# gmum/3d-point-clouds-autocomplete

Hardware: AMD Instinct MI355X
Metric: train-step point-clouds/sec at B=64, N=2048 (Chamfer+EMD) (higher is better)
Workload: dtype f32 storage / accumulation / results; matrix products formed from f16 x2 (bf16 x3) pieces of the fp32 operands — NOT IEEE-fp32 products: the all-fp32-kernel step is `value_strict_fp32`

## Files before the change

3d-point-clouds-autocomplete_amd/csrc/conv_pp.hip:

```cpp
#include "hp_common.h"
#include "hp_conv_split.h"
#include <algorithm>
#include <cstdlib>
#include <type_traits>

namespace {

typedef _Float16 f16x8 __attribute__((ext_vector_type(8)));
typedef _Float16 f16x4 __attribute__((ext_vector_type(4)));
typedef _Float16 f16x2 __attribute__((ext_vector_type(2)));
typedef float f32x16 __attribute__((ext_vector_type(16)));
typedef float f32x4 __attribute__((ext_vector_type(4)));
typedef unsigned int u32x4 __attribute__((ext_vector_type(4)));
typedef unsigned int u32x2 __attribute__((ext_vector_type(2)));

constexpr int kTarget = 14;
constexpr int kExpMax = HP_PP_EXP_MAX;

__device__ __forceinline__ int frexp_exp(unsigned bits) {
    const int E = (int)((bits >> 23) & 0xff);
    return E ? E - 126 : 0;
}
__device__ __forceinline__ float pow2f(int e) {
    e = max(-126, min(127, e));
// ... 356 lines not shown
                        L[q + 1][pr] = s2[1];
                    }
                    if (row < M) {
                        *reinterpret_cast<u32x4*>(line + q * 16) = u32x4{H[q][0], H[q][1], H[q + 1][0], H[q + 1][1]};
                        *reinterpret_cast<u32x4*>(line + 64 + q * 16) = u32x4{L[q][0], L[q][1], L[q + 1][0], L[q + 1][1]};
                    }
                }
            }
        }
        __syncthreads();
    }
}

__global__ __launch_bounds__(256) void conv1_pp_kernel(const float* __restrict__ x, long sXz, const float* __restrict__ W, long sWz,
                                                       const float* __restrict__ b, long sBz, _Float16* __restrict__ h, int* __restrict__ hexp,
                                                       long sWs, long R) {
    __shared__ float smax[4];
    const int z = blockIdx.y;
    x += z * sXz; W += z * sWz; b += z * sBz;
    unsigned char* hb = reinterpret_cast<unsigned char*>(h) + z * sWs * 4;
    hexp += z * sWs;
    const int c4 = (threadIdx.x & 15) * 4;
    float w0[4], w1[4], w2[4], bb[4];
#pragma unroll
    for (int u = 0; u < 4; ++u) {
        w0[u] = W[(c4 + u) * 3];
        w1[u] = W[(c4 + u) * 3 + 1];
        w2[u] = W[(c4 + u) * 3 + 2];
        bb[u] = b[c4 + u];
    }
    for (long tile = blockIdx.x; tile * 128 < R; tile += gridDim.x) {
        const long base = tile * 128 + (threadIdx.x >> 4);
        float xv[8][3];
#pragma unroll
        for (int q = 0; q < 8; ++q) {
            const long row = min(base + 16 * q, R - 1);
            xv[q][0] = x[row * 3];
            xv[q][1] = x[row * 3 + 1];
            xv[q][2] = x[row * 3 + 2];
        }
        float o[8][4];
        float m = 0.f;
#pragma unroll
        for (int q = 0; q < 8; ++q)
#pragma unroll
            for (int u = 0; u < 4; ++u) {
// ... 138 lines not shown

}

bool hp_conv_presplit_enabled() { return g_presplit.get() != 0; }
int hp_conv_pp_ncb(int l) {
    static const int kC[5] = {0, 64, 128, 256, 512};
    return l <= 1 ? 1 : kC[l] / pp_bn(kC[l]);
}
HP_API int hp_conv_presplit_set(int on) { return g_presplit.set(on); }

static inline long pexp_off(int l, long tp) { return hp_conv_pp_exp_offset(l, tp); }

long hp_conv_pp_fmt_offset(long R) { return hp_conv_pp_exp_offset(5, hp_conv_split_tiles_pad(R)); }

int hp_conv_pp_layer1(int n, const float* x, long sXz, const float* W, long sWz, const float* b, long sBz, float* h1, float* area0,
                      long sWs, long R, hipStream_t stream) {
    const long tp = hp_conv_split_tiles_pad(R), blocks = (R + 127) / 128;
    hipLaunchKernelGGL(conv1_pp_kernel, dim3((unsigned)(blocks < 2048 ? blocks : 2048), n), dim3(256), 0, stream, x, sXz, W, sWz, b, sBz,
                       reinterpret_cast<_Float16*>(h1), reinterpret_cast<int*>(area0 + pexp_off(1, tp)), sWs, R);
    HP_RETURN_LAST_ERROR();
}

int hp_conv_pp_layer(int l, int n, const float* X, const float* bias, long sBiasz, float* C, float* area0, long sWs, long M,
                     float* cmax, int* cidx, int group_rows, hipStream_t stream) {
    static const int kRowsL[5] = {0, 128, 384, 896, 1408};
    static const long kWOffL[4] = {0, 8192, 40960, 172032};
    static const int kKL[4] = {64, 128, 256, 512};
    if (l < 2 || l > 5 || M <= 0) return -1;
    const long tp = hp_conv_split_tiles_pad(M);
    PpParams p{};
    p.A = reinterpret_cast<const _Float16*>(X);
    p.aexp = reinterpret_cast<const int*>(area0 + pexp_off(l - 1, tp));
    p.K = kKL[l - 2];
    p.a_ncb = hp_conv_pp_ncb(l - 1);
// ... 117 lines not shown
```

3d-point-clouds-autocomplete_amd/csrc/conv_split.hip:

```cpp
#include "hp_common.h"
#include "hp_conv_split.h"

namespace {

typedef _Float16 f16x8 __attribute__((ext_vector_type(8)));
typedef _Float16 f16x4 __attribute__((ext_vector_type(4)));
typedef float f32x16 __attribute__((ext_vector_type(16)));
typedef float f32x4 __attribute__((ext_vector_type(4)));
typedef unsigned int u32x4 __attribute__((ext_vector_type(4)));

constexpr int BM = 128, BN = 128, BK = 32, ROW = BK;
constexpr int kTarget = 14;

__device__ __forceinline__ int frexp_exp(unsigned bits) {
    const int E = (int)((bits >> 23) & 0xff);
    return E ? E - 126 : 0;
}
__device__ __forceinline__ float pow2f(int e) {
    e = max(-126, min(127, e));
    return __uint_as_float((unsigned)(e + 127) << 23);
}

struct PrepParams {
    const float* W[4];
    long sWz[4];
    _Float16* hl;
    int* wexp;
    unsigned* amax;
    long n_amax;
    long sArea;
    int* fmt;
    int fmt_value;
};
constexpr int kRows[5] = {0, 128, 384, 896, 1408};
constexpr long kWOff[4] = {0, 8192, 40960, 172032};
constexpr int kK[4] = {64, 128, 256, 512};

__global__ __launch_bounds__(256) void conv_split_prep_kernel(const PrepParams p) {
    const int z = blockIdx.y, lane = threadIdx.x & 63;
    const int row = blockIdx.x * 4 + (threadIdx.x >> 6);
    for (long i = (long)blockIdx.x * 256 + threadIdx.x; i < p.n_amax; i += (long)gridDim.x * 256) p.amax[z * p.sArea + i] = 0u;
    if (blockIdx.x == 0 && threadIdx.x == 0) p.fmt[z * p.sArea] = p.fmt_value;
    int l = 0;
    while (l < 3 && row >= kRows[l + 1]) ++l;
    const int n = row - kRows[l], K = kK[l];
    const float* w = p.W[l] + z * p.sWz[l] + (long)n * K;
    float v[8];
    float m = 0.f;
#pragma unroll
    for (int u = 0; u < 8; ++u) {
        const int k = lane + 64 * u;
        v[u] = k < K ? w[k] : 0.f;
        m = fmaxf(m, fabsf(v[u]));
    }
#pragma unroll
    for (int o = 32; o > 0; o >>= 1) m = fmaxf(m, __shfl_xor(m, o, 64));
    const int e = kTarget - frexp_exp(__float_as_uint(m));
    const float s = pow2f(e);
    _Float16* hl = p.hl + 2 * z * p.sArea + 2 * kWOff[l] + (long)n * 2 * K;
#pragma unroll
    for (int u = 0; u < 8; ++u) {
        const int k = lane + 64 * u;
        if (k < K) {
            const float xs = v[u] * s;
            const _Float16 hh = (_Float16)xs;
            hl[(k >> 5) * 64 + (k & 31)] = hh;
            hl[(k >> 5) * 64 + 32 + (k & 31)] = (_Float16)(xs - (float)hh);
        }
    }
    if (lane == 0) p.wexp[z * p.sArea + row] = e;
}

__global__ __launch_bounds__(256) void conv1_kernel(const float* __restrict__ x, long sXz, const float* __restrict__ W, long sWz,
                                                    const float* __restrict__ b, long sBz, float* __restrict__ h, long sHz,
                                                    unsigned* __restrict__ amax, long sAz, long R) {
    __shared__ float smax[4];
    const int z = blockIdx.y;
    x += z * sXz; W += z * sWz; b += z * sBz; h += z * sHz;
    const int c4 = (threadIdx.x & 15) * 4;
    float w0[4], w1[4], w2[4], bb[4];
#pragma unroll
    for (int u = 0; u < 4; ++u) {
        w0[u] = W[(c4 + u) * 3];
        w1[u] = W[(c4 + u) * 3 + 1];
        w2[u] = W[(c4 + u) * 3 + 2];
// ... 278 lines not shown
            out[(k >> 5) * 64 + (k & 31)] = hh;
            out[(k >> 5) * 64 + 32 + (k & 31)] = (_Float16)(xs - (float)hh);
        }
    }
    if (lane == 0) wexp[row] = e;
}

hp::Switch g_split("HP_CONV_SPLIT", 1);

}

long hp_conv_split_area_floats(long R) { return HP_CS_AMAX_OFF + 20 * hp_conv_split_tiles_pad(R) + 4; }
bool hp_conv_split_enabled() { return g_split.get() != 0; }
HP_API int hp_conv_split_set(int on) { return g_split.set(on); }

int hp_conv_split_prep(int n, const float* const* W0, const float* const* W1, float* area0, long sArea, long R, int fmt, hipStream_t stream) {
    PrepParams p{};
    for (int l = 0; l < 4; ++l) {
        p.W[l] = W0[l];
        p.sWz[l] = n > 1 ? (long)(W1[l] - W0[l]) : 0;
    }
    p.amax = reinterpret_cast<unsigned*>(area0 + HP_CS_AMAX_OFF);
    p.n_amax = 4 * hp_conv_split_tiles_pad(R);
    p.wexp = reinterpret_cast<int*>(area0 + HP_CS_WEXP_OFF);
    p.hl = reinterpret_cast<_Float16*>(area0 + HP_CS_HI_OFF);
    p.sArea = sArea;
    p.fmt = reinterpret_cast<int*>(area0 + hp_conv_pp_fmt_offset(R));
    p.fmt_value = fmt;
    hipLaunchKernelGGL(conv_split_prep_kernel, dim3(kRows[4] / 4, n), dim3(256), 0, stream, p);
    HP_RETURN_LAST_ERROR();
}

int hp_conv_split_layer1(int n, const float* x, long sXz, const float* W, long sWz, const float* b, long sBz, float* h1, long sHz,
                         float* area0, long sArea, long R, hipStream_t stream) {
    const long blocks = (R + 127) / 128;
    hipLaunchKernelGGL(conv1_kernel, dim3((unsigned)(blocks < 2048 ? blocks : 2048), n), dim3(256), 0, stream, x, sXz, W, sWz, b,
                       sBz, h1, sHz, reinterpret_cast<unsigned*>(area0 + HP_CS_AMAX_OFF), sArea, R);
    HP_RETURN_LAST_ERROR();
}

int hp_conv_split_layer(int l, int n, const float* X, long sXz, const float* bias, long sBiasz, float* C, long sCz, float* area0,
                        long sArea, long M, int relu, int colmax, float* cmax, int* cidx, int group_rows, hipStream_t stream) {
    if (l < 2 || l > 5 || M <= 0) return -1;
    CsParams p{};
// ... 55 lines not shown
```

3d-point-clouds-autocomplete_amd/csrc/heads_fwd.hip:

```cpp
#include "hp_common.h"
#include <algorithm>
#include <cstdlib>
#include <type_traits>

namespace {

typedef __bf16 bf16x8 __attribute__((ext_vector_type(8)));
typedef float f32x4 __attribute__((ext_vector_type(4)));
typedef unsigned int u32x4 __attribute__((ext_vector_type(4)));

constexpr int kK = 2048, kSteps = kK / 32;
constexpr int kWaves = 5, kThreads = kWaves * 64;
constexpr int kT5Step = 12 * 1024;
constexpr int kG = 2, kStages = kSteps / kG;
constexpr int kT5Ring = 3, kWRing = 4;
constexpr int kT5Stage = kG * kT5Step;
constexpr int kWStage = kWaves * kG * 2048;
constexpr int kLds = kT5Ring * kT5Stage + kWRing * kWStage;
constexpr long kT5Bytes = (long)kSteps * kT5Step;

__device__ __forceinline__ void split3(const float (&x)[8], bf16x8& p1, bf16x8& p2, bf16x8& p3) {
    u32x4 a, b, c;
#pragma unroll
    for (int i = 0; i < 4; ++i) {
        const float x0 = x[2 * i], x1 = x[2 * i + 1];
        const float h0 = __uint_as_float(__float_as_uint(x0) & 0xffff0000u), h1 = __uint_as_float(__float_as_uint(x1) & 0xffff0000u);
        const float r0 = x0 - h0, r1 = x1 - h1;
        const float m0 = __uint_as_float(__float_as_uint(r0) & 0xffff0000u), m1 = __uint_as_float(__float_as_uint(r1) & 0xffff0000u);
        const float s0 = r0 - m0, s1 = r1 - m1;
        a[i] = __builtin_amdgcn_perm(__float_as_uint(x1), __float_as_uint(x0), 0x07060302u);
        b[i] = __builtin_amdgcn_perm(__float_as_uint(r1), __float_as_uint(r0), 0x07060302u);
        c[i] = __builtin_amdgcn_perm(__float_as_uint(s1), __float_as_uint(s0), 0x07060302u);
    }
    p1 = __builtin_bit_cast(bf16x8, a);
    p2 = __builtin_bit_cast(bf16x8, b);
    p3 = __builtin_bit_cast(bf16x8, c);
}

__global__ __launch_bounds__(64) void heads_t5_split_kernel(int B, const float* __restrict__ t5, unsigned char* __restrict__ out) {
    const int s = blockIdx.x >> 2, ct = blockIdx.x & 3, lane = threadIdx.x, c = 16 * ct + (lane & 15), kg = lane >> 4;
    float x[8];
#pragma unroll
    for (int j = 0; j < 8; ++j) x[j] = 0.f;
    if (c < B) {
        const f32x4 v0 = *reinterpret_cast<const f32x4*>(t5 + (long)c * kK + 32 * s + 8 * kg);
        const f32x4 v1 = *reinterpret_cast<const f32x4*>(t5 + (long)c * kK + 32 * s + 8 * kg + 4);
#pragma unroll
        for (int j = 0; j < 4; ++j) {
            x[j] = v0[j];
            x[4 + j] = v1[j];
        }
    }
    bf16x8 p[3];
    split3(x, p[0], p[1], p[2]);
    unsigned char* dst = out + (long)s * kT5Step + (ct * 3) * 1024 + lane * 16;
#pragma unroll
    for (int q = 0; q < 3; ++q) *reinterpret_cast<bf16x8*>(dst + q * 1024) = p[q];
}

__device__ __forceinline__ void glds16(const void* sbase, unsigned voff, unsigned lds_dst) {
    unsigned keep;
// ... 98 lines not shown
    }
    asm volatile("s_waitcnt vmcnt(0)" ::: "memory");
}

hp::Switch g_heads_fwd("HP_HEADS_FWD", 1);

}

bool hp_heads_fwd_enabled() { return g_heads_fwd.get() != 0; }
int hp_heads_fwd_set(int on) { return g_heads_fwd.set(on); }
long hp_heads_fwd_ws_floats() { return kT5Bytes / 4; }
bool hp_heads_fwd_ok(int B, int N, int K, const float* t5, const float* W, const float* ws) {
    auto a16 = [](const void* p) { return (reinterpret_cast<uintptr_t>(p) & 15) == 0; };
    return B >= 1 && B <= 64 && K == kK && N >= 16 && (long)N * K * 4 < (1L << 32) && a16(t5) && a16(W) && a16(ws);
}
int hp_heads_fwd(int B, int N, const float* t5, const float* W, const float* bias, float* theta, int theta_ld, float* ws,
                 hipStream_t stream) {
    unsigned char* t5p = reinterpret_cast<unsigned char*>(ws);
    hipLaunchKernelGGL(heads_t5_split_kernel, dim3(kSteps * 4), dim3(64), 0, stream, B, t5, t5p);
    const int ntiles = (N + 15) / 16;
    const int grid = (ntiles + kWaves - 1) / kWaves;
    hipLaunchKernelGGL(heads_fwd_kernel, dim3(grid), dim3(kThreads), 0, stream, B, N, W, bias, t5p, theta, theta_ld);
    HP_RETURN_LAST_ERROR();
}
```

3d-point-clouds-autocomplete_amd/csrc/hp_conv_split.h:

```cpp
#pragma once
#include <hip/hip_runtime.h>

#define HP_CS_WEXP_OFF 0L
#define HP_CS_HI_OFF 1408L
#define HP_CS_LO_OFF (HP_CS_HI_OFF + 434176L / 2)
#define HP_CS_AMAX_OFF (HP_CS_LO_OFF + 434176L / 2)

#define HP_PP_EXP_MAX 54
#define HP_PP_FMT_F32 0
#define HP_PP_FMT_P 0x50464d54

inline long hp_conv_split_tiles_pad(long R) { return ((R + 127) / 128 + 3) / 4 * 4; }
long hp_conv_split_area_floats(long R);
bool hp_conv_split_enabled();
int hp_conv_split_prep(int n, const float* const* W0, const float* const* W1, float* area0, long sArea, long R, int fmt, hipStream_t stream);
int hp_conv_split_layer1(int n, const float* x, long sXz, const float* W, long sWz, const float* b, long sBz, float* h1, long sHz,
                         float* area0, long sArea, long R, hipStream_t stream);
int hp_conv_split_layer(int l, int n, const float* X, long sXz, const float* bias, long sBiasz, float* C, long sCz, float* area0,
                        long sArea, long M, int relu, int colmax, float* cmax, int* cidx, int group_rows, hipStream_t stream);

bool hp_conv_presplit_enabled();
long hp_conv_pp_fmt_offset(long R);
int hp_conv_pp_layer1(int n, const float* x, long sXz, const float* W, long sWz, const float* b, long sBz, float* h1, float* area0,
                      long sWs, long R, hipStream_t stream);
int hp_conv_pp_layer(int l, int n, const float* X, const float* bias, long sBiasz, float* C, float* area0, long sWs, long M,
                     float* cmax, int* cidx, int group_rows, hipStream_t stream);
int hp_conv_pp_mark(int n, float* area0, long sWs, long R, int fmt, hipStream_t stream);
int hp_conv_pp_unpack_ws(float* ws, long R, hipStream_t stream);
inline long hp_conv_pp_exp_offset(int l, long tp) { return HP_CS_AMAX_OFF + 4 * tp + (long)(l - 1) * 4 * tp; }
int hp_conv_pp_ncb(int l);
```

3d-point-clouds-autocomplete_amd/csrc/hp_model.h:

```cpp
#pragma once

#define HP_MAX_HEADS 8
#define HP_MAX_TN_LAYERS 8

typedef struct HpEncoderWeights {
    const float* conv_w[5];
    const float* conv_b[5];
    const float* fc_w;
    const float* fc_b;
    const float* mu_w;
    const float* mu_b;
    const float* std_w;
    const float* std_b;
} HpEncoderWeights;

typedef struct HpEncoderGrads {
    float* conv_w[5];
    float* conv_b[5];
    float* fc_w;
    float* fc_b;
    float* mu_w;
    float* mu_b;
    float* std_w;
    float* std_b;
// ... 52 lines not shown

enum { HP_HEADS_FWD_STREAM = 0, HP_HEADS_FWD_GEMM = 1, HP_HEADS_FWD_PER_HEAD = 2 };
enum { HP_HEADS_DW_DIRECT = 0, HP_HEADS_DW_GEMM = 1, HP_HEADS_DW_PER_HEAD = 2, HP_HEADS_DW_SKIPPED = 3 };
typedef struct HpHeadsPlan {
    int fwd_route;
    int dw_route;
    int dw_rows_route;
} HpHeadsPlan;

#ifdef __cplusplus
bool hp_heads_dw_fast_ok(int cols, const float* t5, const float* out);
bool hp_heads_fwd_enabled();
int hp_heads_fwd_set(int on);
long hp_heads_fwd_ws_floats();
bool hp_heads_fwd_ok(int B, int N, int K, const float* t5, const float* W, const float* ws);
int hp_heads_fwd(int B, int N, const float* t5, const float* W, const float* bias, float* theta, int theta_ld, float* ws,
                 hipStream_t stream);
int hp_heads_dw_launch(int Kc, int rows, int r0, const float* dtheta, int theta_ld, const float* t5, int cols, float* dW,
                       float* db, hipStream_t stream);
#endif
```

3d-point-clouds-autocomplete_amd/csrc/model.hip:

```cpp
#include "hp_common.h"
#include "hp_gemm.h"
#include "hp_conv_split.h"
#include "hp_model.h"
#include "hp_skinny.h"
#include "hp_enc_bwd.h"
#include <algorithm>
#include <cstdlib>

extern "C" int hp_gemm_f32(const HpGemmDesc* d, hipStream_t stream);
extern "C" int hp_gemm_tile_rows(const HpGemmDesc* d);
extern "C" int hp_colsum_f32(int batch, int M, int N, const float* X, long sXz, int ldx, const float* mask, long sMaskz,
                             int ldmask, float* out, long sOz, float* ws, hipStream_t stream);

namespace {

constexpr int kEnc[6] = {3, 64, 128, 256, 512, 512};
constexpr int kTrunk[5] = {64, 128, 512, 1024, 2048};
constexpr long kSplitWs = 4L << 20;

#define TRY(x)            \
    do {                  \
        int _rc = (x);    \
        if (_rc) return _rc; \
    } while (0)

inline long cdiv(long a, long b) { return (a + b - 1) / b; }

int pick_ksplit(int outM, int outN, int kc, int batch) {
    const long tiles = cdiv(outM, 64) * cdiv(outN, 64) * batch;
    if (tiles >= 512 || kc < 256) return 1;
    long ks = tiles >= 256 ? std::min<long>(cdiv(768, tiles), kc / 512)
                           : std::min<long>(cdiv(512, tiles), kc / 128);
    ks = std::max<long>(1, std::min<long>(ks, (long)outM * outN * batch <= 8192 ? 128 : 64));
    while (ks > 1 && (long)outM * outN * batch * ks > kSplitWs) --ks;
    return (int)ks;
}

struct Op {
    hipStream_t s;
    float* splitws;
    const int* dyn = nullptr;
// ... 300 lines not shown
        }
        __syncthreads();
    }
}

__global__ __launch_bounds__(256) void vae_head_fwd_kernel(long n, const float* __restrict__ eps, const float* __restrict__ mu,
                                                           const float* __restrict__ lv, float* __restrict__ z, int out, int z_ld,
                                                           float* __restrict__ explv) {
    const long t = (long)blockIdx.x * 256 + threadIdx.x;
    if (t >= n) return;
    const float e = expf(lv[t]);
    explv[t] = e;
    z[(t / out) * z_ld + t % out] = __builtin_fmaf(eps[t], e, mu[t]);
}

__global__ __launch_bounds__(256) void vae_head_bwd_kernel(long n, const float* __restrict__ eps, const float* __restrict__ lv,
                                                           const float* __restrict__ gz, int out, int gz_ld,
                                                           const float* __restrict__ gmu, const float* __restrict__ gexplv,
                                                           float* __restrict__ dmu, float* __restrict__ dlv) {
    const long t = (long)blockIdx.x * 256 + threadIdx.x;
    if (t >= n) return;
    const float a = gz ? gz[(t / out) * gz_ld + t % out] : 0.f;
    dmu[t] = a + (gmu ? gmu[t] : 0.f);
    dlv[t] = (a * eps[t] + (gexplv ? gexplv[t] : 0.f)) * expf(lv[t]);
}

long enc_fwd_ws(long B, long Np) { return B * Np * (64 + 128 + 256 + 512 + 512) + hp_conv_split_area_floats(B * Np); }
long enc_bwd_ws(long B, long out) {
    const long Rc = B * 512;
    return Rc * 4 + Rc * (64 + 128 + 256 + 512) * 2 + B * (2 * out + 4 * 512) + kSplitWs + 64 + (B * (5 * 512 + 4) + 16) +
// ... 54 lines not shown
    }
    for (int e = 0; e < n && Sh > 1; ++e) {
        const HpEncoderWeights* w = t[e].w;
        float* hs = t[e].slabs + (long)S * 64 * 512;
        for (int hd = 0; hd < (t[e].is_vae ? 2 : 1); ++hd) {
            HpSkOp& op = pr.op[pr.nops++];
            op.type = HP_SK_FIN; op.phase = 2;
            op.a.p = hs + (long)hd * Sh * 64 * out_size; op.a.slab = 64L * out_size; op.a.S = Sh; op.a.ld = out_size;
            op.a.bias = hd ? w->std_b : w->mu_b;
            op.out = hd ? t[e].lv : t[e].mu; op.out_ld = hd ? out_size : t[e].mu_ld;
            op.M = B; op.N = out_size; op.K = 1;
        }
    }
    return 0;
}
int enc_tail_forward_skinny(int B, int out_size, int n, const EncTail* t, hipStream_t stream) {
    HpSkProgram pr;
    if (enc_tail_forward_program(B, out_size, n, t, pr)) return -2;
    return hp_skinny_run(&pr, stream);
}

struct EncTailBwd {
    const float *g, *f;
    const HpEncoderWeights* w;
    const float* dmu;
    int dmu_ld;
    const float* dlv;
    const HpEncoderGrads* gr;
    float *dfc, *dg, *slabs;
};
int enc_tail_backward_program(int B, int out_size, int n, const EncTailBwd* t, HpSkProgram& pr) {
    if (B > 64 || out_size % 32) return -2;
    pr = HpSkProgram{};
// ... 76 lines not shown
    d5.group_rows = Np;
    r.tr = r.split ? 128 : hp_gemm_tile_rows(&d5);
    r.tail_off = -1;
    r.fused = r.tr > 0 && Np % r.tr == 0;
    if (r.fused) {
        r.tiles = R / r.tr;
        if (R * 512 - up4(2 * r.tiles * 512) >= 4L * 64 * 512 + 8L * 64 * out_size) r.tail_off = up4(2 * r.tiles * 512);
    }
    return r;
}
inline bool enc_fwd_tails_try_skinny(const EncFwdRoute& r, int B) { return hp_skinny_enabled() && r.tail_off >= 0 && B <= 64; }

int encoder_forward_impl(int B, int Np, int out_size, int n, const HpEncoderIO* io, hipStream_t stream) {
    const long R = (long)B * Np;
    const EncFwdRoute route = enc_fwd_route(B, Np, out_size, n);
    Op op{stream, nullptr};
    const HpEncoderIO& e0 = io[0];
    const HpEncoderIO& e1 = io[n - 1];
    auto dz = [&](const float* a0, const float* a1) { return n > 1 ? (long)(a1 - a0) : 0L; };
    float* h[6];
    h[0] = nullptr;
    h[1] = e0.ws;
    for (int l = 2; l <= 5; ++l) h[l] = h[l - 1] + R * kEnc[l - 1];
    const long sWs = dz(e0.ws, e1.ws);
    const bool split = route.split;
    float* area = h[5] + R * 512;
    const bool presplit = route.presplit;
    if (split) {
        const float* W0[4] = {e0.w->conv_w[1], e0.w->conv_w[2], e0.w->conv_w[3], e0.w->conv_w[4]};
        const float* W1[4] = {e1.w->conv_w[1], e1.w->conv_w[2], e1.w->conv_w[3], e1.w->conv_w[4]};
        TRY(hp_conv_split_prep(n, W0, W1, area, sWs, R, presplit ? HP_PP_FMT_P : HP_PP_FMT_F32, stream));
    } else {
        TRY(hp_conv_pp_mark(n, area, sWs, R, HP_PP_FMT_F32, stream));
    }
    if (presplit) {
        TRY(hp_conv_pp_layer1(n, e0.x, dz(e0.x, e1.x), e0.w->conv_w[0], dz(e0.w->conv_w[0], e1.w->conv_w[0]), e0.w->conv_b[0],
                              dz(e0.w->conv_b[0], e1.w->conv_b[0]), h[1], area, sWs, R, stream));
        for (int l = 2; l <= 4; ++l)
            TRY(hp_conv_pp_layer(l, n, h[l - 1], e0.w->conv_b[l - 1], dz(e0.w->conv_b[l - 1], e1.w->conv_b[l - 1]), h[l], area, sWs, R,
                                 nullptr, nullptr, 0, stream));
    } else if (split) {
        TRY(hp_conv_split_layer1(n, e0.x, dz(e0.x, e1.x), e0.w->conv_w[0], dz(e0.w->conv_w[0], e1.w->conv_w[0]), e0.w->conv_b[0],
                                 dz(e0.w->conv_b[0], e1.w->conv_b[0]), h[1], sWs, area, sWs, R, stream));
        for (int l = 2; l <= 4; ++l)
            TRY(hp_conv_split_layer(l, n, h[l - 1], sWs, e0.w->conv_b[l - 1], dz(e0.w->conv_b[l - 1], e1.w->conv_b[l - 1]), h[l], sWs,
                                    area, sWs, R, 1, 0, nullptr, nullptr, 0, stream));
    } else {
        const float* in = e0.x;
        long sIn = dz(e0.x, e1.x);
        for (int l = 1; l <= 4; ++l) {
            TRY(op.lin_fwd(in, sIn, kEnc[l - 1], e0.w->conv_w[l - 1], dz(e0.w->conv_w[l - 1], e1.w->conv_w[l - 1]),
                           e0.w->conv_b[l - 1], dz(e0.w->conv_b[l - 1], e1.w->conv_b[l - 1]), h[l], sWs, kEnc[l], (int)R, kEnc[l],
// ... 23 lines not shown
        else
            TRY(hp_gemm_f32(&d5, stream));
        hipLaunchKernelGGL(colmax_tiles_kernel, dim3(2, B, n), dim3(256), 0, stream, d5.cmax, d5.cidx, Np / tr, tr, 512, io[0].g,
                           io[0].argidx, sWs, io[n - 1].g, io[n - 1].argidx);
    } else {
        if (split)
            TRY(hp_conv_split_layer(5, n, h[4], sWs, d5.bias, d5.sBiasz, h[5], sWs, area, sWs, R, 0, 0, nullptr, nullptr, 0, stream));
        else
            TRY(op.lin_fwd(h[4], sWs, 512, e0.w->conv_w[4], d5.sBz, e0.w->conv_b[4], d5.sBiasz, h[5], sWs, 512, (int)R, 512, 512, n,
                           false));
        for (int z = 0; z < n; ++z)
            hipLaunchKernelGGL(colmax_kernel, dim3(512 / 64, B), dim3(256), 0, stream, h[5] + z * sWs, Np, 512, io[z].g,
                               io[z].argidx);
    }
    int sk = -2;
    if (enc_fwd_tails_try_skinny(route, B)) {
        EncTail t[2];
        for (int z = 0; z < n; ++z) t[z] = EncTail{io[z].g, io[z].w, io[z].is_vae, io[z].f, io[z].mu, io[z].lv, h[5] + z * sWs + tail_off,
                           (!io[z].is_vae && io[z].out_ld > 0) ? io[z].out_ld : out_size};
        sk = enc_tail_forward_skinny(B, out_size, n, t, stream);
    }
    if (sk != -2) TRY(sk);
    for (int z = 0; z < n; ++z) {
        const HpEncoderIO& e = io[z];
        if (sk == -2) {
            TRY(op.lin_fwd(e.g, 0, 512, e.w->fc_w, 0, e.w->fc_b, 0, e.f, 0, 512, B, 512, 512, 1, true));
            TRY(op.lin_fwd(e.f, 0, 512, e.w->mu_w, 0, e.w->mu_b, 0, e.mu, 0, (!e.is_vae && e.out_ld > 0) ? e.out_ld : out_size, B,
                           out_size, 512, 1, false));
            if (e.is_vae)
                TRY(op.lin_fwd(e.f, 0, 512, e.w->std_w, 0, e.w->std_b, 0, e.lv, 0, out_size, B, out_size, 512, 1, false));
        }
        if (e.is_vae) {
            const long nel = (long)B * out_size;
            hipLaunchKernelGGL(vae_head_fwd_kernel, dim3((int)cdiv(nel, 256)), dim3(256), 0, stream, nel, e.eps, e.mu, e.lv, e.z,
                               out_size, e.out_ld > 0 ? e.out_ld : out_size, e.explv);
        }
    }
// ... 289 lines not shown
                                  const float* eps, const int* argidx, const float* g, const float* f, const float* lv,
                                  const float* grad_out, int grad_out_ld, const float* grad_mu, const float* grad_explv,
                                  const HpEncoderGrads* gr, float* ws, const float* fwd_ws, int dedup, hipStream_t stream) {
    const HpEncoderBwdIO io{x, w, eps, argidx, g, f, lv, grad_out, grad_mu, grad_explv, gr, ws, fwd_ws, is_vae, grad_out_ld};
    return encoder_backward_impl(B, Np, out_size, 1, &io, dedup, stream);
}
HP_API int hp_encoder_backward(int B, int Np, const float* x, const HpEncoderWeights* w, int out_size, int is_vae,
                               const float* eps, const int* argidx, const float* g, const float* f, const float* lv,
                               const float* grad_out, const float* grad_mu, const float* grad_explv,
                               const HpEncoderGrads* gr, float* ws, const float* fwd_ws, int dedup, hipStream_t stream) {
    return hp_encoder_backward_ld(B, Np, x, w, out_size, is_vae, eps, argidx, g, f, lv, grad_out, out_size, grad_mu, grad_explv, gr, ws,
                                  fwd_ws, dedup, stream);
}
HP_API int hp_encoder_backward_set_fused(int on) { return g_enc_bwd_fused.set(on); }
HP_API int hp_encoder_backward_set_chain_f16(int on) { return hp_enc_bwd_chain_f16_set(on); }
HP_API int hp_encoder_backward_pair(int B, int Np, int out_size, const HpEncoderBwdIO* io, int dedup, hipStream_t stream) {
    return encoder_backward_impl(B, Np, out_size, 2, io, dedup, stream);
}

HP_API int hp_encoder_plan(int B, int Np, int out_size, int n, const int* is_vae, const int* ld, int aligned, int dedup,
                           HpEncoderPlan* plan) {
    HP_CHECK_ARG(n >= 1 && n <= 2 && is_vae && plan && enc_fwd_shape_ok(B, Np, out_size, n));
    for (int z = 0; z < n; ++z) HP_CHECK_ARG(!ld || ld[z] == 0 || ld[z] >= out_size);
    HP_CHECK_ARG(!dedup || (long)Np * 512 < (1L << 31));
    *plan = HpEncoderPlan{};
    float* const base = reinterpret_cast<float*>(uintptr_t(1) << 40);
    const long span = 1L << 34;
    HpEncoderWeights w{};
    HpEncoderGrads gr{};
    for (int l = 0; l < 5; ++l) {
// ... 41 lines not shown
        const int ok = ask && enc_tail_backward_program(B, out_size, n, t, pr) == 0 && hp_skinny_check(&pr) == 0;
        for (int z = 0; z < n; ++z) plan->bwd_tails_skinny[z] = ok;
    }
    return 0;
}

namespace {
template <typename P>
bool heads_contiguous(P const* hw, P const* hb, const int* out, int n) {
    for (int h = 0; h + 1 < n; ++h)
        if (hw[h + 1] != hw[h] + (long)out[h] * 2048 || hb[h + 1] != hb[h] + out[h]) return false;
    return n > 0;
}

int trunk_forward_skinny(int B, int in_size, const float* latent, const HpHyperWeights* w, float* t, float* slabs,
                         hipStream_t stream) {
    if (B > 64 || in_size % 32) return -2;
    HpSkProgram pr{};
    HpSkSrc src{};
    src.p = latent; src.S = 1; src.ld = in_size;
    float* tl = t;
    float* sl = slabs;
    int kin = in_size;
    for (int l = 0; l < 5; ++l) {
        const int N = kTrunk[l];
        const int S = sk_ranges(kin, N / 32, 4);
        HpSkOp& op = pr.op[pr.nops++];
        op.type = HP_SK_F; op.phase = l;
        op.a = src;
        op.w = w->trunk_w[l]; op.w_ld = kin;
        op.M = B; op.N = N; op.K = kin; op.CL = kin / S;
// ... 6 lines not shown
        } else {
            op.out = sl; op.out_slab = 64L * N;
            next.p = sl; next.slab = 64L * N; next.S = S; next.bias = w->trunk_b[l]; next.relu = l < 4;
            next.mat = tl; next.ldmat = N;
            sl += (long)S * 64 * N;
            if (sl - slabs > kSplitWs) return -2;
        }
        src = next;
        kin = N;
        tl += (long)B * N;
    }
    if (src.S > 1) {
        HpSkOp& op = pr.op[pr.nops++];
        op.type = HP_SK_FIN; op.phase = 5;
        op.out = src.mat; op.out_ld = src.ldmat;
        src.mat = nullptr;
        op.a = src;
        op.M = B; op.N = 2048; op.K = 1;
    }
    return hp_skinny_run(&pr, stream);
}

int trunk_backward_skinny(int B, int in_size, const float* latent, const HpHyperWeights* w, const float* const* act,
                          float* const* dt, const HpHyperGrads* gr, float* grad_latent, float* slabs, hipStream_t stream) {
    if (B > 64 || in_size % 32) return -2;
    HpSkProgram pr{};
    HpSkSrc src{};
    src.p = dt[4]; src.S = 1; src.ld = kTrunk[4];
    float* sl = slabs;
    int phase = 0;
    auto dw_op = [&](int l) {
        HpSkOp& op = pr.op[pr.nops++];
        op.type = HP_SK_W; op.phase = phase;
// ... 80 lines not shown
}
}

HP_API long hp_hypernet_saved_floats(int B) { return (long)B * (64 + 128 + 512 + 1024 + 2048) + kSplitWs + 64; }
HP_API long hp_hypernet_backward_workspace_floats(int B) { return (long)B * (64 + 128 + 512 + 1024 + 2048) + kSplitWs + 64; }

HP_API int hp_hypernet_set_heads_stream(int on) { return hp_heads_fwd_set(on); }

HP_API int hp_hypernet_forward(int B, int in_size, const float* latent, const HpHyperWeights* w, float* t, float* theta,
                               int theta_ld, hipStream_t stream) {
    HP_CHECK_ARG(B > 0 && in_size > 0 && latent && w && t && theta && w->n_heads > 0 && w->n_heads <= HP_MAX_HEADS);
    Op op{stream, hyper_splitws(t, B)};
    const float* in = latent;
    int kin = in_size;
    float* tl = t;
    int sk = hp_skinny_enabled() ? trunk_forward_skinny(B, in_size, latent, w, t, op.splitws, stream) : -2;
    if (sk != -2) {
        TRY(sk);
        in = t + (long)B * (64 + 128 + 512 + 1024);
    } else {
        for (int l = 0; l < 5; ++l) {
            TRY(op.lin_fwd(in, 0, kin, w->trunk_w[l], 0, w->trunk_b[l], 0, tl, 0, kTrunk[l], B, kTrunk[l], kin, 1, l < 4));
            in = tl;
            kin = kTrunk[l];
            tl += (long)B * kTrunk[l];
        }
    }
    const int total = heads_total(w);
    HP_CHECK_ARG(total <= theta_ld);
    switch (heads_fwd_route(B, w, t)) {
    case HP_HEADS_FWD_STREAM:
        TRY(hp_heads_fwd(B, total, in, w->head_w[0], w->head_b[0], theta, theta_ld, op.splitws, stream));
        break;
    case HP_HEADS_FWD_GEMM:
        TRY(op.lin_fwd(in, 0, 2048, w->head_w[0], 0, w->head_b[0], 0, theta, 0, theta_ld, B, total, 2048, 1, false));
        break;
    default: {
        int off = 0;
        for (int hd = 0; hd < w->n_heads; ++hd) {
            TRY(op.lin_fwd(in, 0, 2048, w->head_w[hd], 0, w->head_b[hd], 0, theta + off, 0, theta_ld, B, w->head_out[hd], 2048,
                           1, false));
            off += w->head_out[hd];
        }
    }
    }
    HP_RETURN_LAST_ERROR();
}
// ... 191 lines not shown
```

include/hyperpocket_hip.h:

```cpp
#ifndef HYPERPOCKET_HIP_H
#define HYPERPOCKET_HIP_H

#ifdef __cplusplus
extern "C" {
#endif

typedef struct ihipStream_t* hpStream_t;


int hp_nndistance(int b, int n, const float* xyz, int m, const float* xyz2, float* result, int* result_i,
                  float* result2, int* result2_i, hpStream_t stream);

int hp_nn_set_queries_per_lane(int r);
int hp_nn_queries_per_lane(int b, int n, int m);

int hp_nndistancegrad(int b, int n, const float* xyz1, int m, const float* xyz2, const float* grad_dist1,
                      const int* idx1, const float* grad_dist2, const int* idx2, float* grad_xyz1, float* grad_xyz2,
                      hpStream_t stream);

int hp_approxmatch(int b, int n, int m, const float* xyz1, const float* xyz2, float* match, float* temp,
                   hpStream_t stream);
long hp_approxmatch_workspace_floats(int b, int n, int m);
int hp_approxmatch_ws(int b, int n, int m, const float* xyz1, const float* xyz2, float* match, float* temp, float* ws,
                      hpStream_t stream);
// ... 210 lines not shown
    int dw_route;
    int dw_rows_route;
} HpHeadsPlan;
int hp_hypernet_heads_plan(int B, const HpHyperWeights* w, const HpHyperGrads* grads , const float* t,
                           const float* dW_rows , HpHeadsPlan* plan);

int hp_hypernet_heads_dw_adam(int Kc, int rows, int r0, const float* dtheta_all, int theta_ld, const float* t5_all,
                              float* W_rows, float* m_rows, float* v_rows, float lr, float beta1, float beta2, float eps,
                              int step, hpStream_t stream);
int hp_hypernet_heads_dw_adam_bg(int Kc, int rows, int r0, const float* dtheta_all, int theta_ld, const float* t5_all,
                                 float* W_rows, float* m_rows, float* v_rows, float lr, float beta1, float beta2, float eps,
                                 int step, int cus, hpStream_t stream);

int hp_skinny_set_enabled(int on);
long hp_skinny_programs_run(void);

long hp_target_theta_size(int n_hidden, const int* channels);
long hp_target_saved_floats(int B, int N, int n_hidden, const int* channels);
int hp_target_forward(int B, int N, int n_hidden, const int* channels, const float* theta, int theta_ld, const float* pts,
                      float* acts, float* y, hpStream_t stream);
long hp_target_backward_workspace_floats(int B, int N, int n_hidden, const int* channels);
int hp_target_backward(int B, int N, int n_hidden, const int* channels, const float* theta, int theta_ld, const float* pts,
                       const float* acts, const float* grad_y, float* grad_theta, float* ws, hpStream_t stream);

int hp_target_fused_supported(int n_hidden, const int* channels);
long hp_target_fused_workspace_floats(int B, int N);
int hp_target_fused_set_f16(int on);
int hp_target_fused_forward(int B, int N, const float* theta, int theta_ld, const float* pts, float* y, hpStream_t stream);
int hp_target_fused_backward(int B, int N, const float* theta, int theta_ld, const float* pts, const float* grad_y,
                             float* grad_theta, float* ws, hpStream_t stream);
// ... 161 lines not shown
```

Measured before the change: 28460.

## Fold small prep and finalize launches into neighboring kernels in training step

Three launch-saving folds are added behind a switch mask that defaults to all on. The conv weight hi/lo split prep now runs as extra workgroups appended to the layer-1 conv kernel grid. The encoder tail's final split-K reduction, bias and VAE reparameterization become one batched kernel covering both encoders. The trunk's last split-K finalize is folded into the heads t5 split kernel, which sums the slabs, adds bias and writes t5. The aim is fewer tiny kernel launches and serialization points per step, at the cost of more complex kernels and shared code paths.

After: 28670, median of 6. No clear change (+0.7%).

```diff
diff --git a/3d-point-clouds-autocomplete_amd/csrc/conv_pp.hip b/3d-point-clouds-autocomplete_amd/csrc/conv_pp.hip
--- a/3d-point-clouds-autocomplete_amd/csrc/conv_pp.hip
+++ b/3d-point-clouds-autocomplete_amd/csrc/conv_pp.hip
@@ -1,5 +1,6 @@
 #include "hp_common.h"
 #include "hp_conv_split.h"
+#include "hp_conv_split_wprep.h"
 #include <algorithm>
 #include <cstdlib>
 #include <type_traits>
@@ -394,9 +395,13 @@
 
 __global__ __launch_bounds__(256) void conv1_pp_kernel(const float* __restrict__ x, long sXz, const float* __restrict__ W, long sWz,
                                                        const float* __restrict__ b, long sBz, _Float16* __restrict__ h, int* __restrict__ hexp,
-                                                       long sWs, long R) {
+                                                       long sWs, long R, int tile_wgs, const HpConvPrepParams prep) {
     __shared__ float smax[4];
     const int z = blockIdx.y;
+    if ((int)blockIdx.x >= tile_wgs) {
+        hp_cprep::body(prep, (int)blockIdx.x - tile_wgs, (int)gridDim.x - tile_wgs, z);
+        return;
+    }
     x += z * sXz; W += z * sWz; b += z * sBz;
     unsigned char* hb = reinterpret_cast<unsigned char*>(h) + z * sWs * 4;
     hexp += z * sWs;
@@ -409,7 +414,7 @@
         w2[u] = W[(c4 + u) * 3 + 2];
         bb[u] = b[c4 + u];
     }
-    for (long tile = blockIdx.x; tile * 128 < R; tile += gridDim.x) {
+    for (long tile = blockIdx.x; tile * 128 < R; tile += tile_wgs) {
         const long base = tile * 128 + (threadIdx.x >> 4);
         float xv[8][3];
 #pragma unroll
@@ -578,10 +583,12 @@
 long hp_conv_pp_fmt_offset(long R) { return hp_conv_pp_exp_offset(5, hp_conv_split_tiles_pad(R)); }
 
 int hp_conv_pp_layer1(int n, const float* x, long sXz, const float* W, long sWz, const float* b, long sBz, float* h1, float* area0,
-                      long sWs, long R, hipStream_t stream) {
+                      long sWs, long R, const HpConvPrepParams* prep, hipStream_t stream) {
     const long tp = hp_conv_split_tiles_pad(R), blocks = (R + 127) / 128;
-    hipLaunchKernelGGL(conv1_pp_kernel, dim3((unsigned)(blocks < 2048 ? blocks : 2048), n), dim3(256), 0, stream, x, sXz, W, sWz, b, sBz,
-                       reinterpret_cast<_Float16*>(h1), reinterpret_cast<int*>(area0 + pexp_off(1, tp)), sWs, R);
+    const int tile_wgs = (int)(blocks < 2048 ? blocks : 2048);
+    hipLaunchKernelGGL(conv1_pp_kernel, dim3((unsigned)(tile_wgs + (prep ? hp_cprep::kWgs : 0)), n), dim3(256), 0, stream, x, sXz, W, sWz,
+                       b, sBz, reinterpret_cast<_Float16*>(h1), reinterpret_cast<int*>(area0 + pexp_off(1, tp)), sWs, R, tile_wgs,
+                       prep ? *prep : HpConvPrepParams{});
     HP_RETURN_LAST_ERROR();
 }
 
diff --git a/3d-point-clouds-autocomplete_amd/csrc/conv_split.hip b/3d-point-clouds-autocomplete_amd/csrc/conv_split.hip
--- a/3d-point-clouds-autocomplete_amd/csrc/conv_split.hip
+++ b/3d-point-clouds-autocomplete_amd/csrc/conv_split.hip
@@ -1,5 +1,6 @@
 #include "hp_common.h"
 #include "hp_conv_split.h"
+#include "hp_conv_split_wprep.h"
 
 namespace {
 
@@ -21,54 +22,13 @@
     return __uint_as_float((unsigned)(e + 127) << 23);
 }
 
-struct PrepParams {
-    const float* W[4];
-    long sWz[4];
-    _Float16* hl;
-    int* wexp;
-    unsigned* amax;
-    long n_amax;
-    long sArea;
-    int* fmt;
-    int fmt_value;
-};
-constexpr int kRows[5] = {0, 128, 384, 896, 1408};
-constexpr long kWOff[4] = {0, 8192, 40960, 172032};
-constexpr int kK[4] = {64, 128, 256, 512};
+typedef HpConvPrepParams PrepParams;
+using hp_cprep::kRows;
+using hp_cprep::kWOff;
+using hp_cprep::kK;
 
 __global__ __launch_bounds__(256) void conv_split_prep_kernel(const PrepParams p) {
-    const int z = blockIdx.y, lane = threadIdx.x & 63;
-    const int row = blockIdx.x * 4 + (threadIdx.x >> 6);
-    for (long i = (long)blockIdx.x * 256 + threadIdx.x; i < p.n_amax; i += (long)gridDim.x * 256) p.amax[z * p.sArea + i] = 0u;
-    if (blockIdx.x == 0 && threadIdx.x == 0) p.fmt[z * p.sArea] = p.fmt_value;
-    int l = 0;
-    while (l < 3 && row >= kRows[l + 1]) ++l;
-    const int n = row - kRows[l], K = kK[l];
-    const float* w = p.W[l] + z * p.sWz[l] + (long)n * K;
-    float v[8];
-    float m = 0.f;
-#pragma unroll
-    for (int u = 0; u < 8; ++u) {
-        const int k = lane + 64 * u;
-        v[u] = k < K ? w[k] : 0.f;
-        m = fmaxf(m, fabsf(v[u]));
-    }
-#pragma unroll
-    for (int o = 32; o > 0; o >>= 1) m = fmaxf(m, __shfl_xor(m, o, 64));
-    const int e = kTarget - frexp_exp(__float_as_uint(m));
-    const float s = pow2f(e);
-    _Float16* hl = p.hl + 2 * z * p.sArea + 2 * kWOff[l] + (long)n * 2 * K;
-#pragma unroll
-    for (int u = 0; u < 8; ++u) {
-        const int k = lane + 64 * u;
-        if (k < K) {
-            const float xs = v[u] * s;
-            const _Float16 hh = (_Float16)xs;
-            hl[(k >> 5) * 64 + (k & 31)] = hh;
-            hl[(k >> 5) * 64 + 32 + (k & 31)] = (_Float16)(xs - (float)hh);
-        }
-    }
-    if (lane == 0) p.wexp[z * p.sArea + row] = e;
+    hp_cprep::body(p, (int)blockIdx.x, (int)gridDim.x, (int)blockIdx.y);
 }
 
 __global__ __launch_bounds__(256) void conv1_kernel(const float* __restrict__ x, long sXz, const float* __restrict__ W, long sWz,
@@ -377,7 +337,7 @@
 bool hp_conv_split_enabled() { return g_split.get() != 0; }
 HP_API int hp_conv_split_set(int on) { return g_split.set(on); }
 
-int hp_conv_split_prep(int n, const float* const* W0, const float* const* W1, float* area0, long sArea, long R, int fmt, hipStream_t stream) {
+HpConvPrepParams hp_conv_split_prep_params(int n, const float* const* W0, const float* const* W1, float* area0, long sArea, long R, int fmt) {
     PrepParams p{};
     for (int l = 0; l < 4; ++l) {
         p.W[l] = W0[l];
@@ -390,7 +350,12 @@
     p.sArea = sArea;
     p.fmt = reinterpret_cast<int*>(area0 + hp_conv_pp_fmt_offset(R));
     p.fmt_value = fmt;
-    hipLaunchKernelGGL(conv_split_prep_kernel, dim3(kRows[4] / 4, n), dim3(256), 0, stream, p);
+    return p;
+}
+
+int hp_conv_split_prep(int n, const float* const* W0, const float* const* W1, float* area0, long sArea, long R, int fmt, hipStream_t stream) {
+    const PrepParams p = hp_conv_split_prep_params(n, W0, W1, area0, sArea, R, fmt);
+    hipLaunchKernelGGL(conv_split_prep_kernel, dim3(hp_cprep::kWgs, n), dim3(256), 0, stream, p);
     HP_RETURN_LAST_ERROR();
 }
 
diff --git a/3d-point-clouds-autocomplete_amd/csrc/heads_fwd.hip b/3d-point-clouds-autocomplete_amd/csrc/heads_fwd.hip
--- a/3d-point-clouds-autocomplete_amd/csrc/heads_fwd.hip
+++ b/3d-point-clouds-autocomplete_amd/csrc/heads_fwd.hip
@@ -1,4 +1,5 @@
 #include "hp_common.h"
+#include "hp_skinny.h"
 #include <algorithm>
 #include <cstdlib>
 #include <type_traits>
@@ -37,14 +38,27 @@
     p3 = __builtin_bit_cast(bf16x8, c);
 }
 
-__global__ __launch_bounds__(64) void heads_t5_split_kernel(int B, const float* __restrict__ t5, unsigned char* __restrict__ out) {
+__global__ __launch_bounds__(64) void heads_t5_split_kernel(int B, const float* __restrict__ t5, int S, long slab,
+                                                            const float* __restrict__ bias5, float* __restrict__ t5w,
+                                                            unsigned char* __restrict__ out) {
     const int s = blockIdx.x >> 2, ct = blockIdx.x & 3, lane = threadIdx.x, c = 16 * ct + (lane & 15), kg = lane >> 4;
     float x[8];
 #pragma unroll
     for (int j = 0; j < 8; ++j) x[j] = 0.f;
     if (c < B) {
-        const f32x4 v0 = *reinterpret_cast<const f32x4*>(t5 + (long)c * kK + 32 * s + 8 * kg);
-        const f32x4 v1 = *reinterpret_cast<const f32x4*>(t5 + (long)c * kK + 32 * s + 8 * kg + 4);
+        const long at = (long)c * kK + 32 * s + 8 * kg;
+        f32x4 v0 = *reinterpret_cast<const f32x4*>(t5 + at);
+        f32x4 v1 = *reinterpret_cast<const f32x4*>(t5 + at + 4);
+        if (S > 1) {
+            for (int r = 1; r < S; ++r) {
+                v0 += *reinterpret_cast<const f32x4*>(t5 + r * slab + at);
+                v1 += *reinterpret_cast<const f32x4*>(t5 + r * slab + at + 4);
+            }
+            v0 += *reinterpret_cast<const f32x4*>(bias5 + 32 * s + 8 * kg);
+            v1 += *reinterpret_cast<const f32x4*>(bias5 + 32 * s + 8 * kg + 4);
+            *reinterpret_cast<f32x4*>(t5w + at) = v0;
+            *reinterpret_cast<f32x4*>(t5w + at + 4) = v1;
+        }
 #pragma unroll
         for (int j = 0; j < 4; ++j) {
             x[j] = v0[j];
@@ -173,10 +187,17 @@
     auto a16 = [](const void* p) { return (reinterpret_cast<uintptr_t>(p) & 15) == 0; };
     return B >= 1 && B <= 64 && K == kK && N >= 16 && (long)N * K * 4 < (1L << 32) && a16(t5) && a16(W) && a16(ws);
 }
-int hp_heads_fwd(int B, int N, const float* t5, const float* W, const float* bias, float* theta, int theta_ld, float* ws,
-                 hipStream_t stream) {
+int hp_heads_fwd(int B, int N, const float* t5, const HpSkSrc* t5s, const float* W, const float* bias, float* theta, int theta_ld,
+                 float* ws, hipStream_t stream) {
     unsigned char* t5p = reinterpret_cast<unsigned char*>(ws);
-    hipLaunchKernelGGL(heads_t5_split_kernel, dim3(kSteps * 4), dim3(64), 0, stream, B, t5, t5p);
+    if (t5s && t5s->S > 1) {
+        if (t5s->ld != kK || t5s->ldmat != kK || !t5s->bias || !t5s->mat || t5s->relu || t5s->mask) return -1;
+        hipLaunchKernelGGL(heads_t5_split_kernel, dim3(kSteps * 4), dim3(64), 0, stream, B, t5s->p, t5s->S, t5s->slab, t5s->bias,
+                           t5s->mat, t5p);
+    } else {
+        hipLaunchKernelGGL(heads_t5_split_kernel, dim3(kSteps * 4), dim3(64), 0, stream, B, t5, 1, 0L, (const float*)nullptr,
+                           (float*)nullptr, t5p);
+    }
     const int ntiles = (N + 15) / 16;
     const int grid = (ntiles + kWaves - 1) / kWaves;
     hipLaunchKernelGGL(heads_fwd_kernel, dim3(grid), dim3(kThreads), 0, stream, B, N, W, bias, t5p, theta, theta_ld);
diff --git a/3d-point-clouds-autocomplete_amd/csrc/hp_conv_split.h b/3d-point-clouds-autocomplete_amd/csrc/hp_conv_split.h
--- a/3d-point-clouds-autocomplete_amd/csrc/hp_conv_split.h
+++ b/3d-point-clouds-autocomplete_amd/csrc/hp_conv_split.h
@@ -21,8 +21,9 @@
 
 bool hp_conv_presplit_enabled();
 long hp_conv_pp_fmt_offset(long R);
+struct HpConvPrepParams;
 int hp_conv_pp_layer1(int n, const float* x, long sXz, const float* W, long sWz, const float* b, long sBz, float* h1, float* area0,
-                      long sWs, long R, hipStream_t stream);
+                      long sWs, long R, const HpConvPrepParams* prep, hipStream_t stream);
 int hp_conv_pp_layer(int l, int n, const float* X, const float* bias, long sBiasz, float* C, float* area0, long sWs, long M,
                      float* cmax, int* cidx, int group_rows, hipStream_t stream);
 int hp_conv_pp_mark(int n, float* area0, long sWs, long R, int fmt, hipStream_t stream);
diff --git a/3d-point-clouds-autocomplete_amd/csrc/hp_conv_split_wprep.h b/3d-point-clouds-autocomplete_amd/csrc/hp_conv_split_wprep.h
--- /dev/null
+++ b/3d-point-clouds-autocomplete_amd/csrc/hp_conv_split_wprep.h
@@ -0,0 +1,61 @@
+#pragma once
+#include "hp_conv_split.h"
+
+struct HpConvPrepParams {
+    const float* W[4];
+    long sWz[4];
+    _Float16* hl;
+    int* wexp;
+    unsigned* amax;
+    long n_amax;
+    long sArea;
+    int* fmt;
+    int fmt_value;
+};
+HpConvPrepParams hp_conv_split_prep_params(int n, const float* const* W0, const float* const* W1, float* area0, long sArea, long R, int fmt);
+
+namespace hp_cprep {
+
+constexpr int kRows[5] = {0, 128, 384, 896, 1408};
+constexpr long kWOff[4] = {0, 8192, 40960, 172032};
+constexpr int kK[4] = {64, 128, 256, 512};
+constexpr int kWgs = kRows[4] / 4;
+constexpr int kTarget = 14;
+
+__device__ __forceinline__ void body(const HpConvPrepParams& p, int bx, int nbx, int z) {
+    const int lane = threadIdx.x & 63;
+    const int row = bx * 4 + (threadIdx.x >> 6);
+    for (long i = (long)bx * 256 + threadIdx.x; i < p.n_amax; i += (long)nbx * 256) p.amax[z * p.sArea + i] = 0u;
+    if (bx == 0 && threadIdx.x == 0) p.fmt[z * p.sArea] = p.fmt_value;
+    int l = 0;
+    while (l < 3 && row >= kRows[l + 1]) ++l;
+    const int n = row - kRows[l], K = kK[l];
+    const float* w = p.W[l] + z * p.sWz[l] + (long)n * K;
+    float v[8];
+    float m = 0.f;
+#pragma unroll
+    for (int u = 0; u < 8; ++u) {
+        const int k = lane + 64 * u;
+        v[u] = k < K ? w[k] : 0.f;
+        m = fmaxf(m, fabsf(v[u]));
+    }
+#pragma unroll
+    for (int o = 32; o > 0; o >>= 1) m = fmaxf(m, __shfl_xor(m, o, 64));
+    const int E = (int)((__float_as_uint(m) >> 23) & 0xff);
+    const int e = kTarget - (E ? E - 126 : 0);
+    const float s = __uint_as_float((unsigned)(max(-126, min(127, e)) + 127) << 23);
+    _Float16* hl = p.hl + 2 * z * p.sArea + 2 * kWOff[l] + (long)n * 2 * K;
+#pragma unroll
+    for (int u = 0; u < 8; ++u) {
+        const int k = lane + 64 * u;
+        if (k < K) {
+            const float xs = v[u] * s;
+            const _Float16 hh = (_Float16)xs;
+            hl[(k >> 5) * 64 + (k & 31)] = hh;
+            hl[(k >> 5) * 64 + 32 + (k & 31)] = (_Float16)(xs - (float)hh);
+        }
+    }
+    if (lane == 0) p.wexp[z * p.sArea + row] = e;
+}
+
+}
diff --git a/3d-point-clouds-autocomplete_amd/csrc/hp_model.h b/3d-point-clouds-autocomplete_amd/csrc/hp_model.h
--- a/3d-point-clouds-autocomplete_amd/csrc/hp_model.h
+++ b/3d-point-clouds-autocomplete_amd/csrc/hp_model.h
@@ -90,8 +90,9 @@
 int hp_heads_fwd_set(int on);
 long hp_heads_fwd_ws_floats();
 bool hp_heads_fwd_ok(int B, int N, int K, const float* t5, const float* W, const float* ws);
-int hp_heads_fwd(int B, int N, const float* t5, const float* W, const float* bias, float* theta, int theta_ld, float* ws,
-                 hipStream_t stream);
+struct HpSkSrc;
+int hp_heads_fwd(int B, int N, const float* t5, const HpSkSrc* t5s, const float* W, const float* bias, float* theta, int theta_ld,
+                 float* ws, hipStream_t stream);
 int hp_heads_dw_launch(int Kc, int rows, int r0, const float* dtheta, int theta_ld, const float* t5, int cols, float* dW,
                        float* db, hipStream_t stream);
 #endif
diff --git a/3d-point-clouds-autocomplete_amd/csrc/model.hip b/3d-point-clouds-autocomplete_amd/csrc/model.hip
--- a/3d-point-clouds-autocomplete_amd/csrc/model.hip
+++ b/3d-point-clouds-autocomplete_amd/csrc/model.hip
@@ -1,6 +1,7 @@
 #include "hp_common.h"
 #include "hp_gemm.h"
 #include "hp_conv_split.h"
+#include "hp_conv_split_wprep.h"
 #include "hp_model.h"
 #include "hp_skinny.h"
 #include "hp_enc_bwd.h"
@@ -25,6 +26,9 @@
     } while (0)
 
 inline long cdiv(long a, long b) { return (a + b - 1) / b; }
+
+enum { kFoldWsplit = 1, kFoldEncHead = 2, kFoldT5 = 4, kFoldAll = 7 };
+hp::Switch g_step_folds("HP_STEP_FOLDS", kFoldAll, 0, kFoldAll);
 
 int pick_ksplit(int outM, int outN, int kc, int batch) {
     const long tiles = cdiv(outM, 64) * cdiv(outN, 64) * batch;
@@ -355,6 +359,37 @@
     z[(t / out) * z_ld + t % out] = __builtin_fmaf(eps[t], e, mu[t]);
 }
 
+struct EncTailHead {
+    const float *mu_s, *lv_s;
+    const float *mu_b, *lv_b;
+    const float* eps;
+    float *mu, *lv, *z, *explv;
+    long slab;
+    int S, mu_ld, z_ld;
+};
+struct EncTailHeads {
+    EncTailHead e[2];
+};
+__global__ __launch_bounds__(256) void enc_tail_head_kernel(long n, int out, const EncTailHeads a) {
+    const EncTailHead& h = a.e[blockIdx.y];
+    const long t = (long)blockIdx.x * 256 + threadIdx.x;
+    if (t >= n) return;
+    const long r = t / out;
+    const int c = (int)(t % out);
+    float m = h.mu_s[t];
+    for (int s = 1; s < h.S; ++s) m += h.mu_s[t + s * h.slab];
+    m += h.mu_b[c];
+    h.mu[r * h.mu_ld + c] = m;
+    if (!h.lv) return;
+    float l = h.lv_s[t];
+    for (int s = 1; s < h.S; ++s) l += h.lv_s[t + s * h.slab];
+    l += h.lv_b[c];
+    h.lv[t] = l;
+    const float e = expf(l);
+    h.explv[t] = e;
+    h.z[r * h.z_ld + c] = __builtin_fmaf(h.eps[t], e, m);
+}
+
 __global__ __launch_bounds__(256) void vae_head_bwd_kernel(long n, const float* __restrict__ eps, const float* __restrict__ lv,
                                                            const float* __restrict__ gz, int out, int gz_ld,
                                                            const float* __restrict__ gmu, const float* __restrict__ gexplv,
@@ -439,9 +474,17 @@
     }
     return 0;
 }
-int enc_tail_forward_skinny(int B, int out_size, int n, const EncTail* t, hipStream_t stream) {
+int enc_tail_forward_skinny(int B, int out_size, int n, const EncTail* t, hipStream_t stream, HpSkProgram* fin = nullptr) {
     HpSkProgram pr;
     if (enc_tail_forward_program(B, out_size, n, t, pr)) return -2;
+    if (fin) {
+        fin->nops = 0;
+        if (hp_skinny_check(&pr)) return -2;
+        int first = pr.nops;
+        while (first > 0 && pr.op[first - 1].type == HP_SK_FIN && pr.op[first - 1].phase == 2) --first;
+        for (int o = first; o < pr.nops; ++o) fin->op[fin->nops++] = pr.op[o];
+        pr.nops = first;
+    }
     return hp_skinny_run(&pr, stream);
 }
 
@@ -548,6 +591,7 @@
 int encoder_forward_impl(int B, int Np, int out_size, int n, const HpEncoderIO* io, hipStream_t stream) {
     const long R = (long)B * Np;
     const EncFwdRoute route = enc_fwd_route(B, Np, out_size, n);
+    const int folds = g_step_folds.get();
     Op op{stream, nullptr};
     const HpEncoderIO& e0 = io[0];
     const HpEncoderIO& e1 = io[n - 1];
@@ -560,16 +604,19 @@
     const bool split = route.split;
     float* area = h[5] + R * 512;
     const bool presplit = route.presplit;
+    const bool carry_prep = presplit && (folds & kFoldWsplit);
+    HpConvPrepParams prep{};
     if (split) {
         const float* W0[4] = {e0.w->conv_w[1], e0.w->conv_w[2], e0.w->conv_w[3], e0.w->conv_w[4]};
         const float* W1[4] = {e1.w->conv_w[1], e1.w->conv_w[2], e1.w->conv_w[3], e1.w->conv_w[4]};
-        TRY(hp_conv_split_prep(n, W0, W1, area, sWs, R, presplit ? HP_PP_FMT_P : HP_PP_FMT_F32, stream));
+        if (carry_prep) prep = hp_conv_split_prep_params(n, W0, W1, area, sWs, R, HP_PP_FMT_P);
+        else TRY(hp_conv_split_prep(n, W0, W1, area, sWs, R, presplit ? HP_PP_FMT_P : HP_PP_FMT_F32, stream));
     } else {
         TRY(hp_conv_pp_mark(n, area, sWs, R, HP_PP_FMT_F32, stream));
     }
     if (presplit) {
         TRY(hp_conv_pp_layer1(n, e0.x, dz(e0.x, e1.x), e0.w->conv_w[0], dz(e0.w->conv_w[0], e1.w->conv_w[0]), e0.w->conv_b[0],
-                              dz(e0.w->conv_b[0], e1.w->conv_b[0]), h[1], area, sWs, R, stream));
+                              dz(e0.w->conv_b[0], e1.w->conv_b[0]), h[1], area, sWs, R, carry_prep ? &prep : nullptr, stream));
         for (int l = 2; l <= 4; ++l)
             TRY(hp_conv_pp_layer(l, n, h[l - 1], e0.w->conv_b[l - 1], dz(e0.w->conv_b[l - 1], e1.w->conv_b[l - 1]), h[l], area, sWs, R,
                                  nullptr, nullptr, 0, stream));
@@ -623,13 +670,33 @@
                                io[z].argidx);
     }
     int sk = -2;
+    HpSkProgram fin{};
     if (enc_fwd_tails_try_skinny(route, B)) {
         EncTail t[2];
         for (int z = 0; z < n; ++z) t[z] = EncTail{io[z].g, io[z].w, io[z].is_vae, io[z].f, io[z].mu, io[z].lv, h[5] + z * sWs + tail_off,
                            (!io[z].is_vae && io[z].out_ld > 0) ? io[z].out_ld : out_size};
-        sk = enc_tail_forward_skinny(B, out_size, n, t, stream);
+        sk = enc_tail_forward_skinny(B, out_size, n, t, stream, (folds & kFoldEncHead) ? &fin : nullptr);
     }
     if (sk != -2) TRY(sk);
+    if (sk == 0 && fin.nops) {
+        EncTailHeads a{};
+        int k = 0;
+        for (int z = 0; z < n; ++z) {
+            const HpEncoderIO& e = io[z];
+            EncTailHead& hd = a.e[z];
+            const HpSkOp& m = fin.op[k++];
+            hd.mu_s = m.a.p; hd.mu_b = m.a.bias; hd.slab = m.a.slab; hd.S = m.a.S;
+            hd.mu = m.out; hd.mu_ld = m.out_ld;
+            if (e.is_vae) {
+                const HpSkOp& l = fin.op[k++];
+                hd.lv_s = l.a.p; hd.lv_b = l.a.bias; hd.lv = l.out;
+                hd.eps = e.eps; hd.z = e.z; hd.z_ld = e.out_ld > 0 ? e.out_ld : out_size; hd.explv = e.explv;
+            }
+        }
+        const long nel = (long)B * out_size;
+        hipLaunchKernelGGL(enc_tail_head_kernel, dim3((int)cdiv(nel, 256), n), dim3(256), 0, stream, nel, out_size, a);
+        HP_RETURN_LAST_ERROR();
+    }
     for (int z = 0; z < n; ++z) {
         const HpEncoderIO& e = io[z];
         if (sk == -2) {
@@ -949,6 +1016,7 @@
 }
 HP_API int hp_encoder_backward_set_fused(int on) { return g_enc_bwd_fused.set(on); }
 HP_API int hp_encoder_backward_set_chain_f16(int on) { return hp_enc_bwd_chain_f16_set(on); }
+HP_API int hp_step_folds_set(int mask) { return g_step_folds.set(mask); }
 HP_API int hp_encoder_backward_pair(int B, int Np, int out_size, const HpEncoderBwdIO* io, int dedup, hipStream_t stream) {
     return encoder_backward_impl(B, Np, out_size, 2, io, dedup, stream);
 }
@@ -1020,7 +1088,8 @@
 }
 
 int trunk_forward_skinny(int B, int in_size, const float* latent, const HpHyperWeights* w, float* t, float* slabs,
-                         hipStream_t stream) {
+                         hipStream_t stream, HpSkSrc* last = nullptr, long keep = 0) {
+    if (last) *last = HpSkSrc{};
     if (B > 64 || in_size % 32) return -2;
     HpSkProgram pr{};
     HpSkSrc src{};
@@ -1057,9 +1126,15 @@
         HpSkOp& op = pr.op[pr.nops++];
         op.type = HP_SK_FIN; op.phase = 5;
         op.out = src.mat; op.out_ld = src.ldmat;
+        const HpSkSrc slabs5 = src;
         src.mat = nullptr;
         op.a = src;
         op.M = B; op.N = 2048; op.K = 1;
+        if (last && src.p - slabs >= keep) {
+            if (hp_skinny_check(&pr)) return -2;
+            *last = slabs5;
+            --pr.nops;
+        }
     }
     return hp_skinny_run(&pr, stream);
 }
@@ -1170,7 +1245,12 @@
     const float* in = latent;
     int kin = in_size;
     float* tl = t;
-    int sk = hp_skinny_enabled() ? trunk_forward_skinny(B, in_size, latent, w, t, op.splitws, stream) : -2;
+    const int route = heads_fwd_route(B, w, t);
+    HpSkSrc t5s{};
+    const bool fold_t5 = route == HP_HEADS_FWD_STREAM && (g_step_folds.get() & kFoldT5);
+    int sk = hp_skinny_enabled() ? trunk_forward_skinny(B, in_size, latent, w, t, op.splitws, stream, fold_t5 ? &t5s : nullptr,
+                                                        hp_heads_fwd_ws_floats())
+                                 : -2;
     if (sk != -2) {
         TRY(sk);
         in = t + (long)B * (64 + 128 + 512 + 1024);
@@ -1184,9 +1264,9 @@
     }
     const int total = heads_total(w);
     HP_CHECK_ARG(total <= theta_ld);
-    switch (heads_fwd_route(B, w, t)) {
+    switch (route) {
     case HP_HEADS_FWD_STREAM:
-        TRY(hp_heads_fwd(B, total, in, w->head_w[0], w->head_b[0], theta, theta_ld, op.splitws, stream));
+        TRY(hp_heads_fwd(B, total, in, sk == 0 ? &t5s : nullptr, w->head_w[0], w->head_b[0], theta, theta_ld, op.splitws, stream));
         break;
     case HP_HEADS_FWD_GEMM:
         TRY(op.lin_fwd(in, 0, 2048, w->head_w[0], 0, w->head_b[0], 0, theta, 0, theta_ld, B, total, 2048, 1, false));
diff --git a/include/hyperpocket_hip.h b/include/hyperpocket_hip.h
--- a/include/hyperpocket_hip.h
+++ b/include/hyperpocket_hip.h
@@ -248,6 +248,7 @@
 
 int hp_skinny_set_enabled(int on);
 long hp_skinny_programs_run(void);
+int hp_step_folds_set(int mask);
 
 long hp_target_theta_size(int n_hidden, const int* channels);
 long hp_target_saved_floats(int B, int N, int n_hidden, const int* channels);
```
